# CESNET/UltraGrid

Hardware: AMD Instinct MI355X
Metric: Mpixels/s encode (UYVY->DXT5-YCoCg, 4K) (higher is better)
Workload: dtype f32

## Files before the change

### include/ug_mi355x.h

```cpp
#ifndef UG_MI355X_H
#define UG_MI355X_H

#include <stddef.h>
#include <stdint.h>

#ifdef __cplusplus
extern "C" {
#endif

#define UG_HIP_ABI_VERSION 5

#define UG_HIP_SUCCESS      0
#define UG_HIP_EINVAL     (-1)
#define UG_HIP_EUNSUPP    (-2)
#define UG_HIP_ERUNTIME   (-3)

typedef void *ug_hip_stream_t;

typedef enum {
        UG_PF_NONE = 0,
        UG_PF_RGBA = 1,
        UG_PF_UYVY = 2,
        UG_PF_YUYV = 3,
        UG_PF_RGB  = 4,
// ... 61 lines not shown
                                   float *ms_per_launch);

#define UG_DXT_TIES_EVEN    0
#define UG_DXT_TIES_AWAY    1
#define UG_DXT_TIES_DEFAULT UG_DXT_TIES_EVEN

int ug_hip_dxt_encode(ug_pixfmt_t in, ug_dxt_t out, const void *src_dev, void *dst_dev,
                      int width, int height, int src_pitch, ug_hip_stream_t stream);
int ug_hip_dxt_encode_batch(ug_pixfmt_t in, ug_dxt_t out, const void *src_dev, void *dst_dev,
                            int width, int height, int src_pitch, int frames,
                            size_t src_frame_stride, size_t dst_frame_stride,
                            ug_hip_stream_t stream);
int ug_hip_dxt_encode_batch_ex(ug_pixfmt_t in, ug_dxt_t out, const void *src_dev, void *dst_dev,
                               int width, int height, int src_pitch, int frames,
                               size_t src_frame_stride, size_t dst_frame_stride, int ties,
                               ug_hip_stream_t stream);
size_t ug_hip_dxt_size(ug_dxt_t out, int width, int height);

int ug_hip_rgb_to_dxt1(const void *src, void *out, int size_x, int size_y, ug_hip_stream_t stream);
int ug_hip_yuv_to_dxt1(const void *src, void *out, int size_x, int size_y, ug_hip_stream_t stream);
int ug_hip_rgb_to_dxt6(const void *src, void *out, int size_x, int size_y, ug_hip_stream_t stream);
int ug_hip_yuv_to_dxt6(const void *src, void *out, int size_x, int size_y, ug_hip_stream_t stream);
int ug_hip_yuv422_to_yuv444(const void *src, void *out, int pix_count, ug_hip_stream_t stream);

int ug_hip_dxt_decode(ug_dxt_t in, ug_pixfmt_t out, const void *src_dev, void *dst_dev, int width, int height,
                      int dst_pitch, int rshift, int gshift, int bshift, ug_hip_stream_t stream);
int ug_hip_dxt_decode_ex(ug_dxt_t in, ug_pixfmt_t out, const void *src_dev, void *dst_dev, int width, int height,
                         int dst_pitch, int rshift, int gshift, int bshift, int ties, ug_hip_stream_t stream);
int ug_hip_selftest_dxt_decode(unsigned *mismatches, ug_hip_stream_t stream);
int ug_hip_dxt_decode_debug(int mode, unsigned *flagged_blocks_dev);
int ug_hip_selftest_dxt_encode(unsigned *mismatches, ug_hip_stream_t stream);
int ug_hip_dxt_encode_stats(unsigned long long full_form_waves[2], int reset);
int ug_hip_dxt_encode_stats_ex(unsigned long long *counts, int n, int reset);
typedef struct ug_hip_ldgm ug_hip_ldgm;
int ug_hip_ldgm_stats(const ug_hip_ldgm *s, int *launches, int *copies, int *levels);

int  ug_hip_ldgm_create(int device, int k, int m, const int *pcm, int w_f, ug_hip_ldgm **out);
void ug_hip_ldgm_destroy(ug_hip_ldgm *s);
int  ug_hip_ldgm_encode(ug_hip_ldgm *s, void *buf_dev, int ps, ug_hip_stream_t stream);
int  ug_hip_ldgm_decode(ug_hip_ldgm *s, void *buf_dev, int ps, const uint8_t *received, uint8_t *recovered, int *all_data_known,
                        ug_hip_stream_t stream);
int  ug_hip_ldgm_encode_host(ug_hip_ldgm *s, void *buf_host, int ps, ug_hip_stream_t stream);
int  ug_hip_ldgm_decode_host(ug_hip_ldgm *s, void *buf_host, int ps, const uint8_t *received, uint8_t *recovered, int *all_data_known,
                             ug_hip_stream_t stream);

int ug_hip_pixfmt_supported(ug_pixfmt_t in, ug_pixfmt_t out);
int ug_hip_pixfmt_best(ug_pixfmt_t in, const ug_pixfmt_t *candidates, ug_pixfmt_t *out);
int ug_hip_pixfmt_convert(ug_pixfmt_t in, ug_pixfmt_t out, const void *src_dev, void *dst_dev,
                          int width, int height, int src_pitch, int dst_pitch,
                          int rshift, int gshift, int bshift, ug_hip_stream_t stream);
int ug_hip_pixfmt_convert_batch(ug_pixfmt_t in, ug_pixfmt_t out, const void *src_dev, void *dst_dev, int width, int height,
                                int src_pitch, int dst_pitch, int rshift, int gshift, int bshift, int frames,
                                size_t src_frame_stride, size_t dst_frame_stride, ug_hip_stream_t stream);
int ug_hip_pixfmt_line_func(const char *func, const void *src_dev, void *dst_dev, int width, int height, int src_pitch, int dst_pitch, int dst_len,
                            int rshift, int gshift, int bshift, ug_hip_stream_t stream);
int ug_hip_linesize(ug_pixfmt_t fmt, int width);
int ug_hip_deinterlace_blend(void *frame_dev, size_t linesize, int lines, ug_hip_stream_t stream);
int ug_hip_deinterlace_blend_batch(void *frame_dev, size_t linesize, int lines, int frames, size_t frame_stride, ug_hip_stream_t stream);

struct ug_scale_desc {
        const void *src;
        void       *dst;
        ug_pixfmt_t format;
        int         interlaced_merged;
        int         src_width, src_height, dst_width, dst_height;
        size_t      src_pitch, dst_pitch;
// ... 162 lines not shown
```

### ultragrid_amd/csrc/dxt_encode.hip

```cpp
#include "ug_common.h"

#ifndef UG_DXT_TBUF
#define UG_DXT_TBUF 1
#endif

namespace {

constexpr float kInv255  = 0.00392156862745f;
constexpr float kOffset  = (float) (128.0 / 255.0);
constexpr float kInsetC  = (float) ((8.0 / 255.0) / 16.0);
constexpr float kInsetY  = (float) ((16.0 / 255.0) / 32.0);

__device__ __forceinline__ float clamp01(float v) { return fminf(1.0f, fmaxf(0.0f, v)); }

template <bool AWAY>
__device__ __forceinline__ uint32_t round_u32(float x)
{
        if (!AWAY) {
                return (uint32_t) rintf(x);
        }
        const uint32_t r = (uint32_t) (x + 0.5f);
        return x < 0.5f ? 0u : r;
}

constexpr uint32_t kDiv14Exact = 0x0d800000u;
__device__ __forceinline__ float div14(float x)
{
        constexpr float rc = 1.0f / 14.0f;
        const float q = x * rc;
        const float r = __builtin_fmaf(-q, 14.0f, x);
        return __builtin_fmaf(r, rc, q);
}

// ... 45 lines not shown
        x = (x | (x << 1)) & 0x55555555u;
        return x;
}

#ifndef UG_DXT_NO_FAST_INDEX
#define UG_DXT_FAST_INDEX 1
#else
#define UG_DXT_FAST_INDEX 0
#endif
#ifndef UG_DXT1_FAST_GROUP
#define UG_DXT1_FAST_GROUP 2
#endif
#ifndef UG_DXT5_FAST_GROUP
#define UG_DXT5_FAST_GROUP 4
#endif
#ifndef UG_DXT5_ALPHA_GROUP
#define UG_DXT5_ALPHA_GROUP 8
#endif
#ifndef UG_DXT_PAIR_ZONE
#define UG_DXT_PAIR_ZONE 1
#endif
#ifndef UG_DXT_BITS_INDEX
#define UG_DXT_BITS_INDEX 1
#endif
#ifndef UG_DXT_PAIR_COV
#define UG_DXT_PAIR_COV 1
#endif
#ifndef UG_DXT_POW2_FOLD
#define UG_DXT_POW2_FOLD 1
#endif
#ifndef UG_DXT_PAIR_LINEAR
#define UG_DXT_PAIR_LINEAR 1
#endif
[[maybe_unused]] constexpr float kIndexBias = 8388608.0f;
[[maybe_unused]] constexpr uint32_t kIndexBits = 0x4b000000u;
constexpr uint32_t index_bias_sum(int fields, int shift)
{
        uint32_t s = 0;
        for (int n = 0; n < fields && n * shift < 32; n++) s += kIndexBits << (n * shift);
        return s;
}
__device__ unsigned long long g_full_form_waves[2];
__device__ __forceinline__ void count_full_form(int which)
{
        if ((int) threadIdx.x == __builtin_amdgcn_readfirstlane((int) threadIdx.x)) {
                atomicAdd(&g_full_form_waves[which], 1ull);
        }
}
__device__ unsigned long long g_exact_cov_waves;
__device__ __forceinline__ void count_exact_cov()
{
        if ((int) threadIdx.x == __builtin_amdgcn_readfirstlane((int) threadIdx.x)) {
                atomicAdd(&g_exact_cov_waves, 1ull);
        }
}
constexpr int kPairSlots = 256, kPairSlotStride = 16;
__device__ unsigned long long g_exact_pair_waves[kPairSlots * kPairSlotStride];
__device__ __forceinline__ void count_exact_pair()
{
        if ((int) threadIdx.x == __builtin_amdgcn_readfirstlane((int) threadIdx.x)) {
                const uint32_t slot = ((blockIdx.x + 17u * blockIdx.y + 101u * blockIdx.z) * 4u + threadIdx.y) & (kPairSlots - 1);
                atomicAdd(&g_exact_pair_waves[slot * kPairSlotStride], 1ull);
        }
}
struct IndexTables {
        float *alpha;
        float4 *colour;
};

struct Px16 {
        float a[16], b[16], c[16];
};

__device__ __forceinline__ void yuv_pair_to_rgb(float y0, float y1, float u, float v, Px16 &p, int i)
{
        const float U = u - 0.5f, V = v - 0.5f;
        const float rv = 1.7926f * V, gu = 0.2132f * U, gv = 0.5328f * V, bu = 2.1124f * U;
        const float Y0 = 1.1643f * (y0 - 0.0625f), Y1 = 1.1643f * (y1 - 0.0625f);
        p.a[i] = Y0 + rv;
        p.b[i] = (Y0 - gu) - gv;
        p.c[i] = Y0 + bu;
        p.a[i + 1] = Y1 + rv;
        p.b[i + 1] = (Y1 - gu) - gv;
        p.c[i + 1] = Y1 + bu;
}

__device__ __forceinline__ float byte_f(uint32_t w, int k) { return (float) ((w >> (8 * k)) & 0xffu) * kInv255; }

__device__ __forceinline__ void row_rgb(const uint32_t *w, Px16 &p, int i)
{
        p.a[i + 0] = byte_f(w[0], 0); p.b[i + 0] = byte_f(w[0], 1); p.c[i + 0] = byte_f(w[0], 2);
        p.a[i + 1] = byte_f(w[0], 3); p.b[i + 1] = byte_f(w[1], 0); p.c[i + 1] = byte_f(w[1], 1);
        p.a[i + 2] = byte_f(w[1], 2); p.b[i + 2] = byte_f(w[1], 3); p.c[i + 2] = byte_f(w[2], 0);
        p.a[i + 3] = byte_f(w[2], 1); p.b[i + 3] = byte_f(w[2], 2); p.c[i + 3] = byte_f(w[2], 3);
}

template <int IN>
// ... 293 lines not shown
        }
        __device__ __forceinline__ float samp(int r, int s) const
        {
                return (float) ((w[r][s / 3] >> (10 * (s % 3) + 2)) & 0xffu) * kInv255;
        }
        __device__ __forceinline__ void block(int k, Px16 &p) const
        {
#pragma unroll
                for (int r = 0; r < 4; r++) {
#pragma unroll
                        for (int pr = 0; pr < 2; pr++) {
                                const int s = 8 * k + 4 * pr;
                                yuv_pair_to_rgb(samp(r, s + 1), samp(r, s + 3), samp(r, s), samp(r, s + 2), p, 4 * r + 2 * pr);
                        }
                }
        }
        __device__ __forceinline__ void block_edge(int k, Px16 &p, bool half) const
        {
#pragma unroll
                for (int r = 0; r < 4; r++) {
                        const int s = 8 * k;
                        const float u0 = samp(r, s), y00 = samp(r, s + 1), v0 = samp(r, s + 2), y01 = samp(r, s + 3);
                        yuv_pair_to_rgb(y00, y01, u0, v0, p, 4 * r);
                        const float u1 = half ? u0 : samp(r, s + 4), y10 = half ? y01 : samp(r, s + 5), v1 = half ? v0 : samp(r, s + 6), y11 = half ? y01 : samp(r, s + 7);
                        yuv_pair_to_rgb(y10, y11, u1, v1, p, 4 * r + 2);
                }
        }
};

template <bool AWAY, bool PAIRS>
__device__ __forceinline__ uint4 encode_dxt5ycocg(Px16 &p, const IndexTables &tab)
{
        constexpr bool kFold = UG_DXT_POW2_FOLD;
#pragma unroll
        for (int i = 0; i < 16; i++) {
                const float r = p.a[i], g = p.b[i], b = p.c[i];
                const float t = __builtin_fmaf(g, 2.0f, r);
                p.a[i] = kFold ? t + b : (t + b) * 0.25f;
                p.b[i] = __builtin_fmaf(r - b, 0.5f, kOffset);
                p.c[i] = __builtin_fmaf(__builtin_fmaf(g, 2.0f, -r) - b, 0.25f, kOffset);
        }
        float *Y = p.a, *Co = p.b, *Cg = p.c;

        float mnY = Y[0], mxY = Y[0], mnCo = Co[0], mxCo = Co[0], mnCg = Cg[0], mxCg = Cg[0];
#pragma unroll
        for (int i = 1; i < 16; i++) {
                mnY = fminf(mnY, Y[i]);    mxY = fmaxf(mxY, Y[i]);
                mnCo = fminf(mnCo, Co[i]); mxCo = fmaxf(mxCo, Co[i]);
                mnCg = fminf(mnCg, Cg[i]); mxCg = fmaxf(mxCg, Cg[i]);
        }

        if constexpr (!(PAIRS && UG_DXT_PAIR_COV)) {
                const float midx = (mxCo + mnCo) * 0.5f, midy = (mxCg + mnCg) * 0.5f;
                float cov = 0.0f;
#pragma unroll
                for (int i = 0; i < 16; i++) {
                        const float tx = Co[i] - midx, ty = Cg[i] - midy;
                        cov = cov + tx * ty;
                }
                if (cov < 0.0f) {
                        const float t = mxCg; mxCg = mnCg; mnCg = t;
                }
        } else {
                const float midx = (mxCo + mnCo) * 0.5f, midy = (mxCg + mnCg) * 0.5f;
                const float hx = mxCo - mnCo, hy = mxCg - mnCg;
                float rough = 0.0f;
#pragma unroll
                for (int i = 0; i < 16; i += 2) {
                        rough = __builtin_fmaf(Co[i] - midx, Cg[i] - midy, rough);
                }
                const lanemask_t certain = LANEMASK(fabsf(rough) > 0.5e-5f * __builtin_fmaf(hx, hy, hx + hy)) | LANEMASK(hx * hy == 0.0f);
                bool swap;
                if (__builtin_expect(certain == LANEMASK(true), 1)) {
                        swap = rough < 0.0f;
                } else {
                        float mx = midx, my = midy;
                        asm volatile("; exact covariance" : "+v"(mx), "+v"(my) :: "memory");
                        count_exact_cov();
                        float cov = 0.0f;
#pragma unroll
                        for (int i = 0; i < 16; i++) {
                                const float tx = Co[i] - mx, ty = Cg[i] - my;
                                cov = cov + tx * ty;
                        }
                        swap = cov < 0.0f;
                }
                if (swap) {
                        const float t = mxCg; mxCg = mnCg; mnCg = t;
                }
        }

        uint32_t scale = 1;
        float fs = 1.0f, rfs = 1.0f;
        {
                const float m0 = fmaxf(fabsf(mnCo - kOffset), fabsf(mnCg - kOffset));
                const float m1 = fmaxf(fabsf(mxCo - kOffset), fabsf(mxCg - kOffset));
                const float m = fmaxf(m0, m1);
                if (m < (float) (64.0 / 255.0)) { scale = 2; fs = 2.0f; rfs = 0.5f; }
                if (m < (float) (32.0 / 255.0)) { scale = 4; fs = 4.0f; rfs = 0.25f; }
        }

        uint32_t w_end;
        float cmx[2], cmn[2];
        {
                const float q[2] = { 31.0f, 63.0f };
                const float mx_in[2] = { mxCo, mxCg }, mn_in[2] = { mnCo, mnCg };
                uint32_t imax[2], imin[2];
#pragma unroll
                for (int k = 0; k < 2; k++) {
                        float a = kFold ? __builtin_fmaf(mx_in[k] - kOffset, fs, kOffset) : (mx_in[k] - kOffset) * fs + kOffset;
                        float b = kFold ? __builtin_fmaf(mn_in[k] - kOffset, fs, kOffset) : (mn_in[k] - kOffset) * fs + kOffset;
                        const float inset = kFold ? __builtin_fmaf(a - b, 0.0625f, -kInsetC) : (a - b) * 0.0625f - kInsetC;
                        b = clamp01(b + inset);
                        a = clamp01(a - inset);
                        imax[k] = round_u32<AWAY>(a * q[k]);
                        imin[k] = round_u32<AWAY>(b * q[k]);
                }
                w_end = ((imax[0] << 11) | (imax[1] << 5) | (scale - 1)) |
                        (((imin[0] << 11) | (imin[1] << 5) | (scale - 1)) << 16);
                imax[0] = (imax[0] << 3) | (imax[0] >> 2);
                imax[1] = (imax[1] << 2) | (imax[1] >> 4);
                imin[0] = (imin[0] << 3) | (imin[0] >> 2);
                imin[1] = (imin[1] << 2) | (imin[1] >> 4);
                const float inv255 = (float) (1.0 / 255.0);
#pragma unroll
                for (int k = 0; k < 2; k++) {
                        cmx[k] = kFold ? __builtin_fmaf((float) imax[k] * inv255 - kOffset, rfs, kOffset) : ((float) imax[k] * inv255 - kOffset) * rfs + kOffset;
                        cmn[k] = kFold ? __builtin_fmaf((float) imin[k] * inv255 - kOffset, rfs, kOffset) : ((float) imin[k] * inv255 - kOffset) * rfs + kOffset;
                }
        }

        if constexpr (kFold) {
                const float inset = __builtin_fmaf(mxY - mnY, 0.0078125f, -kInsetY);
                mnY = clamp01(__builtin_fmaf(mnY, 0.25f, inset));
                mxY = clamp01(__builtin_fmaf(mxY, 0.25f, -inset));
        } else {
                const float inset = (mxY - mnY) * 0.03125f - kInsetY;
                mnY = clamp01(mnY + inset);
                mxY = clamp01(mxY - inset);
        }
        uint32_t w0 = (round_u32<AWAY>(mnY * 255.0f) << 8) | round_u32<AWAY>(mxY * 255.0f);
        uint32_t w1 = 0;
        {
                const float inv7 = (float) (1.0 / 7.0);
                const float range = mxY - mnY;
#ifdef UG_DXT_IEEE_DIV14
                const float mid = range / 14.0f;
#else
                float mid = div14(range);
                if (__builtin_expect(__any((__float_as_uint(range) - 1u) < (kDiv14Exact - 1u)), 0)) {
                        mid = range / 14.0f;
                }
#endif
                float ab[8];
                if constexpr (kFold) {
                        ab[1] = __builtin_fmaf(mid, 4.0f, mnY * 4.0f);
#pragma unroll
                        for (int k = 2; k <= 7; k++) {
                                const float cx_ = (float) (4 * (8 - k)), cn_ = (float) (4 * (k - 1));
                                const float sum = k <= 3 || k == 5 ? __builtin_fmaf(mnY, cn_, cx_ * mxY) : __builtin_fmaf(mxY, cx_, cn_ * mnY);
                                ab[k] = __builtin_fmaf(mid, 4.0f, sum * inv7);
// ... 89 lines not shown
                                for (int k = 1; k <= 7; k++) {
                                        c += (a <= ab[k]) ? 1u : 0u;
                                }
                                uint32_t &acc = i >= 10 ? hi : lo;
                                acc = (acc << 3) | c;
                        }
                }
                auto map_fields = [](uint32_t w) {
                        const uint32_t M = 0x09249249u;
                        const uint32_t c0 = w & M, c1 = (w >> 1) & M, c2 = (w >> 2) & M;
                        const uint32_t t = c1 & c0;
                        const uint32_t i0 = ((c0 ^ M) & (c1 | c2)) | (t & c2);
                        const uint32_t i1 = c1 ^ c0, i2 = c2 ^ t;
                        return i0 | (i1 << 1) | (i2 << 2);
                };
                lo = map_fields(lo);
                hi = map_fields(hi);
                w0 |= lo << 16;
                w1 = (lo >> 16) | (hi << 14);
        }
        uint32_t w_cidx = 0;
        {
                const float q1 = (float) (1.0 / 3.0), q2 = (float) (2.0 / 3.0);
                const float w1 = 1.0f - q1, w2 = 1.0f - q2;
                float cx[4], cy[4];
                cx[0] = cmx[0]; cy[0] = cmx[1];
                cx[1] = cmn[0]; cy[1] = cmn[1];
                cx[2] = lerp_w(cx[0], cx[1], w1, q1); cy[2] = lerp_w(cy[0], cy[1], w1, q1);
                cx[3] = lerp_w(cx[0], cx[1], w2, q2); cy[3] = lerp_w(cy[0], cy[1], w2, q2);
#if UG_DXT_FAST_INDEX
                const float vx = cx[1] - cx[0], vy = cy[1] - cy[0];
                const float vv = vx * vx + vy * vy;
                const float e0 = fmaxf(fmaxf(mxCo, cx[0]), cx[1]) - fminf(fminf(mnCo, cx[0]), cx[1]);
                const float e1 = fmaxf(fmaxf(fmaxf(mxCg, mnCg), cy[0]), cy[1]) - fminf(fminf(fminf(mxCg, mnCg), cy[0]), cy[1]);
                const float dmax = e0 * e0 + e1 * e1;
                const bool flat = (mnCo == mxCo) & (mnCg == mxCg);
                if (__builtin_expect(__all(((vv >= 1e-5f) & (vv * 256.0f > dmax)) | flat), 1)) {
                        float4 *const tc = tab.colour;
                        constexpr bool kLinear = PAIRS && UG_DXT_PAIR_ZONE && UG_DXT_PAIR_LINEAR;
                        auto write_rows = [&](float ax, float ay, float bx, float by, float cx2, float cy2, float cx3, float cy3) {
                                tc[0 * 64] = make_float4(ax, ay, cx2, cy2);
                                tc[1 * 64] = make_float4(cx2, cy2, cx3, cy3);
                                tc[2 * 64] = make_float4(bx, by, cx3, cy3);
                        };
                        if constexpr (kLinear) {
                                auto linear_row = [&](int a, int b) {
                                        const float mx = cx[a] - cx[b], my = cy[a] - cy[b], sx = cx[a] + cx[b], sy = cy[a] + cy[b];
                                        return make_float4(mx, my, 0.5f * __builtin_fmaf(mx, sx, my * sy), 0.0f);
                                };
                                tc[0 * 64] = linear_row(0, 2);
                                tc[1 * 64] = linear_row(2, 3);
                                tc[2 * 64] = linear_row(1, 3);
                        } else {
                                write_rows(cx[0], cy[0], cx[1], cy[1], cx[2], cy[2], cx[3], cy[3]);
                        }
#if UG_DXT_BITS_INDEX
                        const float inv = 1.5f * __builtin_amdgcn_rcpf(vv);
                        const float ka = vx * inv, kb = vy * inv;
                        const float kc = kFold ? __builtin_fmaf(-cx[0], ka, __builtin_fmaf(-cy[0], kb, -0.25f)) : -(cx[0] * ka + cy[0] * kb) - 0.25f;
#else
                        const float inv = __builtin_amdgcn_rcpf(vv);
                        const float ka = vx * inv, kb = vy * inv;
                        const float kc = -(cx[0] * ka + cy[0] * kb);
#endif
                        uint32_t zones = 0, open = 0;
                        constexpr int kC = UG_DXT5_FAST_GROUP, kGroups = 16 / kC;
                        constexpr int kP = PAIRS && UG_DXT_PAIR_ZONE ? 2 : 1;
// ... 37 lines not shown
                                        } else {
                                                const float ax = Co[i] - q.x, ay = Cg[i] - q.y, bx = Co[i] - q.z, by = Cg[i] - q.w;
                                                const float da = ax * ax + ay * ay, db = bx * bx + by * by;
                                                if (j % kP == 0) {
                                                        zones = (zones << (2 * kP)) + kk[slot][j / kP];
                                                }
                                                open = shift_in(open, LANEMASK(da > db));
                                        }
                                }
                                if constexpr (kLinear) {
                                        static_assert(kC / kP == 2, "two pairs per group");
                                        least = fminf(fminf(least, mag[0]), mag[1]);
                                }
                                __builtin_amdgcn_sched_barrier(0);
                        }
#if UG_DXT_BITS_INDEX
                        zones -= index_bias_sum(16 / kP, 2 * kP);
#endif
                        if (kP == 2) {
                                zones |= zones << 2;
                        }
                        uint32_t c;
                        if constexpr (kLinear) {
                                const float eps = __builtin_fmaf(dmax, 4.76837158203125e-07f, 1e-6f * __builtin_amdgcn_sqrtf(vv));
                                const lanemask_t certain = LANEMASK(least > eps) | LANEMASK(flat);
                                if (__builtin_expect(certain == LANEMASK(true), 1)) {
                                        c = (open | (open << 12)) & 0x000f000fu;
                                        c = (c | (c << 6)) & 0x03030303u;
                                        c = (c | (c << 3)) & 0x11111111u;
                                        c |= c << 2;
                                } else {
                                        asm volatile("; per-pixel distances" ::: "memory");
                                        count_exact_pair();
                                        write_rows(cx[0], cy[0], cx[1], cy[1], cx[2], cy[2], cx[3], cy[3]);
                                        open = 0;
#pragma unroll
                                        for (int i = 15; i >= 0; i--) {
                                                const float4 q = *(const float4 *) ((const char *) tc + (((zones >> (2 * i)) & 3u) << 10));
                                                const float ax = Co[i] - q.x, ay = Cg[i] - q.y, bx = Co[i] - q.z, by = Cg[i] - q.w;
                                                const float da = ax * ax + ay * ay, db = bx * bx + by * by;
                                                open = shift_in(open, LANEMASK(da > db));
                                        }
                                        c = spread16(open);
                                }
                        } else {
                                c = spread16(open);
                        }
                        const uint32_t k0 = zones & 0x55555555u, k1 = (zones >> 1) & 0x55555555u;
                        w_cidx = ((k0 & c) | k1) | ((k0 | c) << 1);
                        if (__any(flat)) {
                                asm volatile("; flat blocks" ::: "memory");
                                float4 p02, p13;
                                if constexpr (kLinear) {
                                        p02 = make_float4(cx[0], cy[0], cx[2], cy[2]); p13 = make_float4(cx[1], cy[1], cx[3], cy[3]);
                                } else {
                                        p02 = tc[0 * 64]; p13 = tc[2 * 64];
                                }
                                const float px[4] = { p02.x, p13.x, p02.z, p13.z }, py[4] = { p02.y, p13.y, p02.w, p13.w };
                                float d[4];
#pragma unroll
                                for (int k = 0; k < 4; k++) {
                                        const float tx = Co[0] - px[k], ty = Cg[0] - py[k];
                                        d[k] = tx * tx + ty * ty;
                                }
                                w_cidx = flat ? palette_index(d[0], d[1], d[2], d[3]) * 0x55555555u : w_cidx;
                        }
                } else
#endif
                {
                asm volatile("; colour index full form" ::: "memory");
#if UG_DXT_FAST_INDEX
                count_full_form(0);
#endif
                f32x2 cx2[4], cy2[4];
#pragma unroll
                for (int k = 0; k < 4; k++) {
                        cx2[k] = (f32x2) { cx[k], cx[k] };
                        cy2[k] = (f32x2) { cy[k], cy[k] };
                }
#pragma unroll
                for (int i = 14; i >= 0; i -= 2) {
                        const f32x2 co = { Co[i], Co[i + 1] }, cg = { Cg[i], Cg[i + 1] };
                        f32x2 d[4];
#pragma unroll
                        for (int k = 0; k < 4; k++) {
                                const f32x2 tx = co - cx2[k], ty = cg - cy2[k];
                                d[k] = tx * tx + ty * ty;
                        }
#pragma unroll
                        for (int h = 1; h >= 0; h--) {
                                const float d0 = d[0][h], d1 = d[1][h], d2 = d[2][h], d3 = d[3][h];
                                const lanemask_t b0 = LANEMASK(d0 > d3), b1 = LANEMASK(d1 > d2), b2 = LANEMASK(d0 > d2),
                                                 b3 = LANEMASK(d1 > d3), b4 = LANEMASK(d2 > d3);
                                w_cidx = shift_in(w_cidx, (b1 & b2) | (b0 & b3));
                                w_cidx = shift_in(w_cidx, b0 & b4);
                        }
                }
                }
        }

        return make_uint4(w0, w1, w_end, w_cidx);
}

template <bool AWAY>
__device__ __forceinline__ uint2 encode_dxt1(const Px16 &p, const IndexTables &tab)
{
// ... 451 lines not shown
                           int src_pitch, int frames, size_t sfs, size_t dfs, int iters, ug_hip_stream_t stream,
                           float *ms_per_launch)
{
        if (!ms_per_launch || iters <= 0) return UG_HIP_EINVAL;
        hipStream_t st = (hipStream_t) stream;
        int rc = ug_hip_dxt_encode_batch(in, out, src, dst, width, height, src_pitch, frames, sfs, dfs, stream);
        if (rc != UG_HIP_SUCCESS) return rc;
        hipEvent_t e0, e1;
        UG_HIP_TRY(hipEventCreate(&e0));
        UG_HIP_TRY(hipEventCreate(&e1));
        {
                (void) hipEventRecord(e0, st);
                for (int i = 0; i < iters && rc == UG_HIP_SUCCESS; i++) {
                        rc = ug_hip_dxt_encode_batch(in, out, src, dst, width, height, src_pitch, frames, sfs, dfs, stream);
                }
                (void) hipEventRecord(e1, st);
                hipError_t e = hipEventSynchronize(e1);
                if (e != hipSuccess) {
                        ug::set_last_error(e, "hipEventSynchronize");
                        rc = UG_HIP_ERUNTIME;
                } else {
                        float ms = 0;
                        (void) hipEventElapsedTime(&ms, e0, e1);
                        *ms_per_launch = ms / iters;
                }
        }
        (void) hipEventDestroy(e0);
        (void) hipEventDestroy(e1);
        return rc;
}

}

extern "C" int ug_hip_dxt_encode_stats(unsigned long long full_form_waves[2], int reset)
{
        UG_HIP_TRY(hipDeviceSynchronize());
        if (full_form_waves) {
                UG_HIP_TRY(hipMemcpyFromSymbol(full_form_waves, HIP_SYMBOL(g_full_form_waves), 2 * sizeof(unsigned long long)));
        }
        if (reset) {
                const unsigned long long zero[2] = { 0, 0 };
                UG_HIP_TRY(hipMemcpyToSymbol(HIP_SYMBOL(g_full_form_waves), zero, sizeof zero));
                UG_HIP_TRY(hipMemcpyToSymbol(HIP_SYMBOL(g_exact_cov_waves), zero, sizeof zero[0]));
                static const unsigned long long no_pairs[kPairSlots * kPairSlotStride] = {};
                UG_HIP_TRY(hipMemcpyToSymbol(HIP_SYMBOL(g_exact_pair_waves), no_pairs, sizeof no_pairs));
        }
        return UG_HIP_SUCCESS;
}

extern "C" int ug_hip_dxt_encode_stats_ex(unsigned long long *counts, int n, int reset)
{
        if (n < 0 || n > 4 || (n > 0 && !counts)) return UG_HIP_EINVAL;
        unsigned long long all[4] = { 0, 0, 0, 0 };
        UG_HIP_TRY(hipDeviceSynchronize());
        if (n > 0) {
                UG_HIP_TRY(hipMemcpyFromSymbol(all, HIP_SYMBOL(g_full_form_waves), 2 * sizeof all[0]));
                UG_HIP_TRY(hipMemcpyFromSymbol(all + 2, HIP_SYMBOL(g_exact_cov_waves), sizeof all[0]));
                static unsigned long long pairs[kPairSlots * kPairSlotStride];
                UG_HIP_TRY(hipMemcpyFromSymbol(pairs, HIP_SYMBOL(g_exact_pair_waves), sizeof pairs));
                for (int i = 0; i < kPairSlots; i++) all[3] += pairs[i * kPairSlotStride];
                for (int i = 0; i < n; i++) counts[i] = all[i];
        }
        return reset ? ug_hip_dxt_encode_stats(nullptr, 1) : UG_HIP_SUCCESS;
}

extern "C" int ug_hip_selftest_dxt_encode(unsigned *mismatches, ug_hip_stream_t stream)
{
        if (!mismatches) return UG_HIP_EINVAL;
        unsigned *dev = nullptr;
        UG_HIP_TRY(hipMalloc((void **) &dev, sizeof *dev));
        hipStream_t st = (hipStream_t) stream;
        hipError_t err = hipMemsetAsync(dev, 0, sizeof *dev, st);
        if (err == hipSuccess) {
                hipLaunchKernelGGL(selftest_div14_kernel, dim3((0x3f800000u >> 8) + 1), dim3(256), 0, st, dev);
                err = hipGetLastError();
        }
        if (err == hipSuccess) err = hipMemcpyAsync(mismatches, dev, sizeof *dev, hipMemcpyDeviceToHost, st);
        if (err == hipSuccess) err = hipStreamSynchronize(st);
        (void) hipFree(dev);
        if (err != hipSuccess) {
                ug::set_last_error(err, "ug_hip_selftest_dxt_encode");
                return UG_HIP_ERUNTIME;
        }
        return UG_HIP_SUCCESS;
}
```

### ultragrid_amd/lib.py

```python
from __future__ import annotations

import ctypes as C
import os

_HERE = os.path.dirname(os.path.abspath(__file__))
LIB_PATH = os.environ.get("UG_MI355X_LIB") or os.path.join(_HERE, "libug_mi355x.so")

PF_NONE, PF_RGBA, PF_UYVY, PF_YUYV, PF_RGB, PF_BGR, PF_V210, PF_RG48, PF_YUV444, PF_UYVY_RAW, PF_I420 = range(11)
PF_R10K, PF_R12L, PF_Y216, PF_Y416, PF_VUYA, PF_DVS10 = range(11, 17)
PF_UYVY_GL = 17
PF_NAMES = {"RGBA": PF_RGBA, "UYVY": PF_UYVY, "YUYV": PF_YUYV, "RGB": PF_RGB, "BGR": PF_BGR, "v210": PF_V210,
            "RG48": PF_RG48, "YUV444": PF_YUV444, "UYVY_RAW": PF_UYVY_RAW, "R10k": PF_R10K, "R12L": PF_R12L, "Y216": PF_Y216,
            "Y416": PF_Y416, "VUYA": PF_VUYA, "DVS10": PF_DVS10}
DXT1, DXT1_YUV, DXT5_YCOCG = 1, 2, 6
TIES_EVEN, TIES_AWAY = 0, 1
JPEG_CS_ASIS, JPEG_CS_RGB, JPEG_CS_YCBCR_BT601, JPEG_CS_YCBCR_BT601_256LVLS, JPEG_CS_YCBCR_BT709 = 0, 1, 2, 3, 4
JPEG_NONINTERLEAVED = 1
JPEG_INPUT_UYVY = 2
JPEG_INPUT_RGB = 4
COPY_NO_WAIT, COPY_NO_JOIN = 1, 2
ABI_VERSION = 5

SUCCESS, EINVAL, EUNSUPP, ERUNTIME = 0, -1, -2, -3

# ... 29 lines not shown
    "ug_hip_device_numa_node": (_i, [_i, C.POINTER(_i)]),
    "ug_hip_bind_thread_to_device": (_i, [_i, C.POINTER(_i)]),
    "ug_hip_numa_node_of_pci": (_i, [C.c_char_p, C.c_char_p, C.POINTER(_i)]),
    "ug_hip_bind_thread_to_numa_node": (_i, [_i, C.c_char_p, C.POINTER(_i)]),
    "ug_hip_time_dxt_encode": (_i, [_i, _i, _vp, _vp, _i, _i, _i, _i, _sz, _sz, _i, _vp, C.POINTER(C.c_float)]),
    "ug_hip_dxt_encode": (_i, [_i, _i, _vp, _vp, _i, _i, _i, _vp]),
    "ug_hip_dxt_encode_batch": (_i, [_i, _i, _vp, _vp, _i, _i, _i, _i, _sz, _sz, _vp]),
    "ug_hip_dxt_encode_batch_ex": (_i, [_i, _i, _vp, _vp, _i, _i, _i, _i, _sz, _sz, _i, _vp]),
    "ug_hip_dxt_size": (_sz, [_i, _i, _i]),
    "ug_hip_rgb_to_dxt1": (_i, [_vp, _vp, _i, _i, _vp]),
    "ug_hip_yuv_to_dxt1": (_i, [_vp, _vp, _i, _i, _vp]),
    "ug_hip_rgb_to_dxt6": (_i, [_vp, _vp, _i, _i, _vp]),
    "ug_hip_yuv_to_dxt6": (_i, [_vp, _vp, _i, _i, _vp]),
    "ug_hip_yuv422_to_yuv444": (_i, [_vp, _vp, _i, _vp]),
    "ug_hip_dxt_decode": (_i, [_i, _i, _vp, _vp, _i, _i, _i, _i, _i, _i, _vp]),
    "ug_hip_dxt_decode_ex": (_i, [_i, _i, _vp, _vp, _i, _i, _i, _i, _i, _i, _i, _vp]),
    "ug_hip_pixfmt_supported": (_i, [_i, _i]),
    "ug_hip_pixfmt_convert": (_i, [_i, _i, _vp, _vp, _i, _i, _i, _i, _i, _i, _i, _vp]),
    "ug_hip_pixfmt_convert_batch": (_i, [_i, _i, _vp, _vp, _i, _i, _i, _i, _i, _i, _i, _i, _sz, _sz, _vp]),
    "ug_hip_linesize": (_i, [_i, _i]),
    "ug_hip_deinterlace_blend": (_i, [_vp, _sz, _i, _vp]),
    "ug_hip_deinterlace_blend_batch": (_i, [_vp, _sz, _i, _i, _sz, _vp]),
    "ug_hip_uyvy_to_i420": (_i, [_vp, _i, _vp, _i, _vp, _i, _vp, _i, _i, _i, _vp]),
    "ug_hip_v210_to_p010le": (_i, [_vp, _i, _vp, _i, _vp, _i, _i, _i, _vp]),
    "ug_hip_yuv420p_to_uyvy": (_i, [_vp, _i, _vp, _i, _vp, _i, _vp, _i, _i, _i, _vp]),
    "ug_hip_yuv422p_to_uyvy": (_i, [_vp, _i, _vp, _i, _vp, _i, _vp, _i, _i, _i, _vp]),
    "ug_hip_yuv422p10le_to_v210": (_i, [_vp, _i, _vp, _i, _vp, _i, _vp, _i, _i, _i, _vp]),
    "ug_hip_uyvy_to_i422": (_i, [_vp, _i, _vp, _i, _vp, _i, _vp, _i, _i, _i, _vp]),
    "ug_hip_selftest_dxt_decode": (_i, [C.POINTER(C.c_uint), _vp]),
    "ug_hip_dxt_decode_debug": (_i, [_i, _vp]),
    "ug_hip_selftest_dxt_encode": (_i, [C.POINTER(C.c_uint), _vp]),
    "ug_hip_dxt_encode_stats": (_i, [C.POINTER(C.c_ulonglong), _i]),
    "ug_hip_dxt_encode_stats_ex": (_i, [C.POINTER(C.c_ulonglong), _i, _i]),
    "ug_hip_ldgm_stats": (_i, [_vp, C.POINTER(_i), C.POINTER(_i), C.POINTER(_i)]),
    "ug_hip_ldgm_create": (_i, [_i, _i, _i, _vp, _i, C.POINTER(_vp)]),
    "ug_hip_ldgm_destroy": (None, [_vp]),
    "ug_hip_ldgm_encode": (_i, [_vp, _vp, _i, _vp]),
    "ug_hip_ldgm_decode": (_i, [_vp, _vp, _i, _vp, _vp, C.POINTER(_i), _vp]),
    "ug_hip_ldgm_encode_host": (_i, [_vp, _vp, _i, _vp]),
    "ug_hip_ldgm_decode_host": (_i, [_vp, _vp, _i, _vp, _vp, C.POINTER(_i), _vp]),
    "ug_hip_uyvy_to_nv12": (_i, [_vp, _i, _vp, _i, _vp, _i, _i, _i, _vp]),
    "ug_hip_pixfmt_best": (_i, [_i, C.POINTER(_i), C.POINTER(_i)]),
    "ug_hip_pixfmt_line_func": (_i, [C.c_char_p, _vp, _vp, _i, _i, _i, _i, _i, _i, _i, _i, _vp]),
    "ug_hip_from_planar": (_i, [C.c_char_p, _vp, _vp]),
    "ug_hip_to_planar": (_i, [C.c_char_p, _vp, _vp]),
    "ug_hip_from_planar_supported": (_i, [C.c_char_p]),
    "ug_hip_to_planar_supported": (_i, [C.c_char_p]),
    "ug_hip_uv_to_av": (_i, [C.c_char_p, C.c_char_p, _vp, _vp, _vp]),
    "ug_hip_av_to_uv": (_i, [C.c_char_p, C.c_char_p, _vp, _i, _vp, C.POINTER(_i), _vp]),
    "ug_hip_uv_to_av_supported": (_i, [C.c_char_p, C.c_char_p]),
    "ug_hip_av_to_uv_supported": (_i, [C.c_char_p, C.c_char_p]),
    "ug_hip_color_coeffs": (_i, [_i, _i, C.POINTER(_i)]),
    "ug_hip_compute_color_coeffs": (_i, [C.c_double, C.c_double, _i, C.POINTER(_i)]),
    "ug_hip_jpeg_qtable": (None, [_i, _i, _vp]),
    "ug_hip_jpeg_divisors": (None, [_vp, _vp]),
    "ug_hip_jpeg_fdct_quant_plane": (_i, [_vp, _i, _i, _i, _i, _i, _vp, _vp, _vp, _vp]),
    "ug_hip_uyvy_to_jpeg420_coeffs": (_i, [_vp, _i, _i, _i, _vp, _vp, _vp, _vp, _vp]),
    "ug_hip_uyvy_to_jpeg422_coeffs": (_i, [_vp, _i, _i, _i, _vp, _vp, _vp, _vp, _vp]),
    "ug_hip_uyvy_to_jpeg42x_coeffs_batch": (_i, [_i, _vp, _i, _i, _i, _vp, _vp, _vp, _vp, _i, _sz, _sz, _sz, _vp]),
    "ug_hip_jpeg_encoder_create": (_i, [_i, _i, _i, _i, C.POINTER(_vp)]),
    "ug_hip_jpeg_encoder_create_sub": (_i, [_i, _i, _i, _i, _i, C.POINTER(_vp)]),
    "ug_hip_jpeg_encoder_create_ex": (_i, [_i, _i, _i, _i, _i, _i, _i, C.POINTER(_vp)]),
    "ug_hip_jpeg_colour_matrix": (_i, [_i, _i, C.POINTER(C.c_float)]),
    "ug_hip_jpeg_colour_convert": (_i, [_i, _i, _i, _vp, _i, _vp, _i, _i, _i, _vp]),
    "ug_hip_jpeg_encoder_destroy": (None, [_vp]),
    "ug_hip_jpeg_encoder_max_size": (_sz, [_vp]),
# ... 75 lines not shown
```

Before: 960,600.

## Derive DXT5-YCoCg chroma box from even pixels with certified fallback to full box

For the paired DXT5-YCoCg path, the colour conversion defers the Co/Cg offset and scale on odd pixels, and the chroma bounding box, diagonal and scale are computed from the eight even pixels only. A certification mask checks margins on the covariance sign, the scale thresholds and endpoint rounding ties. Any wave with an uncertain lane finishes the odd pixels and recomputes the full sixteen-pixel box, diagonal and endpoints, and the later exact paths also finalise the odd pixels on demand. The wave counters are also sharded into strided slots to reduce atomic contention. This cuts min/max and FMA work in the common case, at the cost of extra branches, register pressure and a correctness dependence on the tolerance constants.

```diff
diff --git a/include/ug_mi355x.h b/include/ug_mi355x.h
--- a/include/ug_mi355x.h
+++ b/include/ug_mi355x.h
@@ -117,6 +117,7 @@
 int ug_hip_selftest_dxt_encode(unsigned *mismatches, ug_hip_stream_t stream);
 int ug_hip_dxt_encode_stats(unsigned long long full_form_waves[2], int reset);
 int ug_hip_dxt_encode_stats_ex(unsigned long long *counts, int n, int reset);
+int ug_hip_dxt_encode_stats_box(unsigned long long *waves, int reset);
 typedef struct ug_hip_ldgm ug_hip_ldgm;
 int ug_hip_ldgm_stats(const ug_hip_ldgm *s, int *launches, int *copies, int *levels);
 
diff --git a/ultragrid_amd/csrc/dxt_encode.hip b/ultragrid_amd/csrc/dxt_encode.hip
--- a/ultragrid_amd/csrc/dxt_encode.hip
+++ b/ultragrid_amd/csrc/dxt_encode.hip
@@ -1,4 +1,5 @@
 #include "ug_common.h"
+#include <type_traits>
 
 #ifndef UG_DXT_TBUF
 #define UG_DXT_TBUF 1
@@ -110,6 +111,10 @@
 #ifndef UG_DXT_PAIR_LINEAR
 #define UG_DXT_PAIR_LINEAR 1
 #endif
+#ifndef UG_DXT_PAIR_BOX
+#define UG_DXT_PAIR_BOX 1
+#endif
+[[maybe_unused]] constexpr float kBoxTie = 1.2e-6f, kBoxScale = 2e-6f, kBoxSpread = 4e-6f;
 [[maybe_unused]] constexpr float kIndexBias = 8388608.0f;
 [[maybe_unused]] constexpr uint32_t kIndexBits = 0x4b000000u;
 constexpr uint32_t index_bias_sum(int fields, int shift)
@@ -118,6 +123,23 @@
         for (int n = 0; n < fields && n * shift < 32; n++) s += kIndexBits << (n * shift);
         return s;
 }
+constexpr int kPairSlots = 256, kPairSlotStride = 16;
+constexpr int kWaveCounter = kPairSlots * kPairSlotStride;
+__device__ __forceinline__ void count_wave(unsigned long long *counter)
+{
+        if ((int) threadIdx.x == __builtin_amdgcn_readfirstlane((int) threadIdx.x)) {
+                const uint32_t slot = ((blockIdx.x + 17u * blockIdx.y + 101u * blockIdx.z) * 4u + (uint32_t) __builtin_amdgcn_readfirstlane((int) threadIdx.y)) & (kPairSlots - 1);
+                atomicAdd(&counter[slot * kPairSlotStride], 1ull);
+        }
+}
+#if UG_DXT_PAIR_BOX
+__device__ unsigned long long g_full_form_waves[2][kWaveCounter];
+__device__ __forceinline__ void count_full_form(int which) { count_wave(g_full_form_waves[which]); }
+__device__ unsigned long long g_exact_cov_waves[kWaveCounter];
+__device__ __forceinline__ void count_exact_cov() { count_wave(g_exact_cov_waves); }
+__device__ unsigned long long g_exact_pair_waves[kWaveCounter];
+__device__ __forceinline__ void count_exact_pair() { count_wave(g_exact_pair_waves); }
+#else
 __device__ unsigned long long g_full_form_waves[2];
 __device__ __forceinline__ void count_full_form(int which)
 {
@@ -132,7 +154,6 @@
                 atomicAdd(&g_exact_cov_waves, 1ull);
         }
 }
-constexpr int kPairSlots = 256, kPairSlotStride = 16;
 __device__ unsigned long long g_exact_pair_waves[kPairSlots * kPairSlotStride];
 __device__ __forceinline__ void count_exact_pair()
 {
@@ -141,6 +162,9 @@
                 atomicAdd(&g_exact_pair_waves[slot * kPairSlotStride], 1ull);
         }
 }
+#endif
+__device__ unsigned long long g_box_waves[kWaveCounter];
+[[maybe_unused]] __device__ __forceinline__ void count_box() { count_wave(g_box_waves); }
 struct IndexTables {
         float *alpha;
         float4 *colour;
@@ -500,24 +524,90 @@
 __device__ __forceinline__ uint4 encode_dxt5ycocg(Px16 &p, const IndexTables &tab)
 {
         constexpr bool kFold = UG_DXT_POW2_FOLD;
+        constexpr bool kBox = PAIRS && UG_DXT_PAIR_BOX && UG_DXT_PAIR_COV && UG_DXT_PAIR_ZONE && UG_DXT_PAIR_LINEAR && UG_DXT_FAST_INDEX;
 #pragma unroll
         for (int i = 0; i < 16; i++) {
                 const float r = p.a[i], g = p.b[i], b = p.c[i];
                 const float t = __builtin_fmaf(g, 2.0f, r);
                 p.a[i] = kFold ? t + b : (t + b) * 0.25f;
-                p.b[i] = __builtin_fmaf(r - b, 0.5f, kOffset);
-                p.c[i] = __builtin_fmaf(__builtin_fmaf(g, 2.0f, -r) - b, 0.25f, kOffset);
+                if (!kBox || i % 2 == 0) {
+                        p.b[i] = __builtin_fmaf(r - b, 0.5f, kOffset);
+                        p.c[i] = __builtin_fmaf(__builtin_fmaf(g, 2.0f, -r) - b, 0.25f, kOffset);
+                } else {
+                        p.b[i] = r - b;
+                        p.c[i] = __builtin_fmaf(g, 2.0f, -r) - b;
+                }
         }
         float *Y = p.a, *Co = p.b, *Cg = p.c;
+        [[maybe_unused]] bool have_odd = !kBox;
+        [[maybe_unused]] auto need_odd = [&]() {
+                if constexpr (kBox) {
+                        if (!have_odd) {
+#pragma unroll
+                                for (int i = 1; i < 16; i += 2) {
+                                        Co[i] = __builtin_fmaf(Co[i], 0.5f, kOffset);
+                                        Cg[i] = __builtin_fmaf(Cg[i], 0.25f, kOffset);
+                                }
+                                have_odd = true;
+                        }
+                }
+        };
 
         float mnY = Y[0], mxY = Y[0], mnCo = Co[0], mxCo = Co[0], mnCg = Cg[0], mxCg = Cg[0];
 #pragma unroll
         for (int i = 1; i < 16; i++) {
                 mnY = fminf(mnY, Y[i]);    mxY = fmaxf(mxY, Y[i]);
-                mnCo = fminf(mnCo, Co[i]); mxCo = fmaxf(mxCo, Co[i]);
-                mnCg = fminf(mnCg, Cg[i]); mxCg = fmaxf(mxCg, Cg[i]);
-        }
-
+                if (!kBox || i % 2 == 0) {
+                        mnCo = fminf(mnCo, Co[i]); mxCo = fmaxf(mxCo, Co[i]);
+                        mnCg = fminf(mnCg, Cg[i]); mxCg = fmaxf(mxCg, Cg[i]);
+                }
+        }
+
+        if constexpr (kBox) {
+                asm volatile("" : "+v"(mnY), "+v"(mxY));
+        }
+
+        [[maybe_unused]] lanemask_t box_certain = LANEMASK(true);
+        [[maybe_unused]] lanemask_t luma_flat_certain = 0;
+        [[maybe_unused]] float loCg = mnCg, hiCg = mxCg;
+        [[maybe_unused]] auto pair_diagonal = [&](auto on_even_box) {
+                if constexpr (kBox) {
+                        constexpr bool kEvenBox = decltype(on_even_box)::value;
+                        const float midx = (mxCo + mnCo) * 0.5f, midy = (mxCg + mnCg) * 0.5f;
+                        const float hx = mxCo - mnCo, hy = mxCg - mnCg;
+                        float rough = 0.0f;
+#pragma unroll
+                        for (int i = 0; i < 16; i += 2) {
+                                rough = __builtin_fmaf(Co[i] - midx, Cg[i] - midy, rough);
+                        }
+                        bool swap;
+                        if constexpr (kEvenBox) {
+                                const lanemask_t decided = LANEMASK(fabsf(rough) > 0.5e-5f * __builtin_fmaf(hx, hy, hx + hy));
+                                box_certain = decided & LANEMASK(fminf(hx, hy) > kBoxSpread);
+                                luma_flat_certain = LANEMASK(mnY == mxY) & (decided | LANEMASK(hx * hy == 0.0f));
+                                swap = rough < 0.0f;
+                        } else {
+                                const lanemask_t certain = LANEMASK(fabsf(rough) > 0.5e-5f * __builtin_fmaf(hx, hy, hx + hy)) | LANEMASK(hx * hy == 0.0f);
+                                if (__builtin_expect(certain == LANEMASK(true), 1)) {
+                                        swap = rough < 0.0f;
+                                } else {
+                                        float mx = midx, my = midy;
+                                        asm volatile("; exact covariance" : "+v"(mx), "+v"(my) :: "memory");
+                                        count_exact_cov();
+                                        float cov = 0.0f;
+#pragma unroll
+                                        for (int i = 0; i < 16; i++) {
+                                                const float tx = Co[i] - mx, ty = Cg[i] - my;
+                                                cov = cov + tx * ty;
+                                        }
+                                        swap = cov < 0.0f;
+                                }
+                        }
+                        if (swap) {
+                                const float t = mxCg; mxCg = mnCg; mnCg = t;
+                        }
+                }
+        };
         if constexpr (!(PAIRS && UG_DXT_PAIR_COV)) {
                 const float midx = (mxCo + mnCo) * 0.5f, midy = (mxCg + mnCg) * 0.5f;
                 float cov = 0.0f;
@@ -530,71 +620,136 @@
                         const float t = mxCg; mxCg = mnCg; mnCg = t;
                 }
         } else {
-                const float midx = (mxCo + mnCo) * 0.5f, midy = (mxCg + mnCg) * 0.5f;
-                const float hx = mxCo - mnCo, hy = mxCg - mnCg;
-                float rough = 0.0f;
-#pragma unroll
-                for (int i = 0; i < 16; i += 2) {
-                        rough = __builtin_fmaf(Co[i] - midx, Cg[i] - midy, rough);
-                }
-                const lanemask_t certain = LANEMASK(fabsf(rough) > 0.5e-5f * __builtin_fmaf(hx, hy, hx + hy)) | LANEMASK(hx * hy == 0.0f);
-                bool swap;
-                if (__builtin_expect(certain == LANEMASK(true), 1)) {
-                        swap = rough < 0.0f;
+                if constexpr (kBox) {
+                        pair_diagonal(std::true_type());
                 } else {
-                        float mx = midx, my = midy;
-                        asm volatile("; exact covariance" : "+v"(mx), "+v"(my) :: "memory");
-                        count_exact_cov();
-                        float cov = 0.0f;
-#pragma unroll
-                        for (int i = 0; i < 16; i++) {
-                                const float tx = Co[i] - mx, ty = Cg[i] - my;
-                                cov = cov + tx * ty;
-                        }
-                        swap = cov < 0.0f;
-                }
-                if (swap) {
-                        const float t = mxCg; mxCg = mnCg; mnCg = t;
+                        const float midx = (mxCo + mnCo) * 0.5f, midy = (mxCg + mnCg) * 0.5f;
+                        const float hx = mxCo - mnCo, hy = mxCg - mnCg;
+                        float rough = 0.0f;
+#pragma unroll
+                        for (int i = 0; i < 16; i += 2) {
+                                rough = __builtin_fmaf(Co[i] - midx, Cg[i] - midy, rough);
+                        }
+                        const lanemask_t certain = LANEMASK(fabsf(rough) > 0.5e-5f * __builtin_fmaf(hx, hy, hx + hy)) | LANEMASK(hx * hy == 0.0f);
+                        bool swap;
+                        if (__builtin_expect(certain == LANEMASK(true), 1)) {
+                                swap = rough < 0.0f;
+                        } else {
+                                float mx = midx, my = midy;
+                                asm volatile("; exact covariance" : "+v"(mx), "+v"(my) :: "memory");
+                                count_exact_cov();
+                                float cov = 0.0f;
+#pragma unroll
+                                for (int i = 0; i < 16; i++) {
+                                        const float tx = Co[i] - mx, ty = Cg[i] - my;
+                                        cov = cov + tx * ty;
+                                }
+                                swap = cov < 0.0f;
+                        }
+                        if (swap) {
+                                const float t = mxCg; mxCg = mnCg; mnCg = t;
+                        }
                 }
         }
 
         uint32_t scale = 1;
         float fs = 1.0f, rfs = 1.0f;
-        {
-                const float m0 = fmaxf(fabsf(mnCo - kOffset), fabsf(mnCg - kOffset));
-                const float m1 = fmaxf(fabsf(mxCo - kOffset), fabsf(mxCg - kOffset));
-                const float m = fmaxf(m0, m1);
-                if (m < (float) (64.0 / 255.0)) { scale = 2; fs = 2.0f; rfs = 0.5f; }
-                if (m < (float) (32.0 / 255.0)) { scale = 4; fs = 4.0f; rfs = 0.25f; }
-        }
-
         uint32_t w_end;
         float cmx[2], cmn[2];
-        {
-                const float q[2] = { 31.0f, 63.0f };
-                const float mx_in[2] = { mxCo, mxCg }, mn_in[2] = { mnCo, mnCg };
-                uint32_t imax[2], imin[2];
-#pragma unroll
-                for (int k = 0; k < 2; k++) {
-                        float a = kFold ? __builtin_fmaf(mx_in[k] - kOffset, fs, kOffset) : (mx_in[k] - kOffset) * fs + kOffset;
-                        float b = kFold ? __builtin_fmaf(mn_in[k] - kOffset, fs, kOffset) : (mn_in[k] - kOffset) * fs + kOffset;
-                        const float inset = kFold ? __builtin_fmaf(a - b, 0.0625f, -kInsetC) : (a - b) * 0.0625f - kInsetC;
-                        b = clamp01(b + inset);
-                        a = clamp01(a - inset);
-                        imax[k] = round_u32<AWAY>(a * q[k]);
-                        imin[k] = round_u32<AWAY>(b * q[k]);
-                }
-                w_end = ((imax[0] << 11) | (imax[1] << 5) | (scale - 1)) |
-                        (((imin[0] << 11) | (imin[1] << 5) | (scale - 1)) << 16);
-                imax[0] = (imax[0] << 3) | (imax[0] >> 2);
-                imax[1] = (imax[1] << 2) | (imax[1] >> 4);
-                imin[0] = (imin[0] << 3) | (imin[0] >> 2);
-                imin[1] = (imin[1] << 2) | (imin[1] >> 4);
-                const float inv255 = (float) (1.0 / 255.0);
-#pragma unroll
-                for (int k = 0; k < 2; k++) {
-                        cmx[k] = kFold ? __builtin_fmaf((float) imax[k] * inv255 - kOffset, rfs, kOffset) : ((float) imax[k] * inv255 - kOffset) * rfs + kOffset;
-                        cmn[k] = kFold ? __builtin_fmaf((float) imin[k] * inv255 - kOffset, rfs, kOffset) : ((float) imin[k] * inv255 - kOffset) * rfs + kOffset;
+        if constexpr (!kBox) {
+                {
+                        const float m0 = fmaxf(fabsf(mnCo - kOffset), fabsf(mnCg - kOffset));
+                        const float m1 = fmaxf(fabsf(mxCo - kOffset), fabsf(mxCg - kOffset));
+                        const float m = fmaxf(m0, m1);
+                        if (m < (float) (64.0 / 255.0)) { scale = 2; fs = 2.0f; rfs = 0.5f; }
+                        if (m < (float) (32.0 / 255.0)) { scale = 4; fs = 4.0f; rfs = 0.25f; }
+                }
+                {
+                        const float q[2] = { 31.0f, 63.0f };
+                        const float mx_in[2] = { mxCo, mxCg }, mn_in[2] = { mnCo, mnCg };
+                        uint32_t imax[2], imin[2];
+#pragma unroll
+                        for (int k = 0; k < 2; k++) {
+                                float a = kFold ? __builtin_fmaf(mx_in[k] - kOffset, fs, kOffset) : (mx_in[k] - kOffset) * fs + kOffset;
+                                float b = kFold ? __builtin_fmaf(mn_in[k] - kOffset, fs, kOffset) : (mn_in[k] - kOffset) * fs + kOffset;
+                                const float inset = kFold ? __builtin_fmaf(a - b, 0.0625f, -kInsetC) : (a - b) * 0.0625f - kInsetC;
+                                b = clamp01(b + inset);
+                                a = clamp01(a - inset);
+                                imax[k] = round_u32<AWAY>(a * q[k]);
+                                imin[k] = round_u32<AWAY>(b * q[k]);
+                        }
+                        w_end = ((imax[0] << 11) | (imax[1] << 5) | (scale - 1)) |
+                                (((imin[0] << 11) | (imin[1] << 5) | (scale - 1)) << 16);
+                        imax[0] = (imax[0] << 3) | (imax[0] >> 2);
+                        imax[1] = (imax[1] << 2) | (imax[1] >> 4);
+                        imin[0] = (imin[0] << 3) | (imin[0] >> 2);
+                        imin[1] = (imin[1] << 2) | (imin[1] >> 4);
+                        const float inv255 = (float) (1.0 / 255.0);
+#pragma unroll
+                        for (int k = 0; k < 2; k++) {
+                                cmx[k] = kFold ? __builtin_fmaf((float) imax[k] * inv255 - kOffset, rfs, kOffset) : ((float) imax[k] * inv255 - kOffset) * rfs + kOffset;
+                                cmn[k] = kFold ? __builtin_fmaf((float) imin[k] * inv255 - kOffset, rfs, kOffset) : ((float) imin[k] * inv255 - kOffset) * rfs + kOffset;
+                        }
+                }
+        } else {
+                auto scale_and_end_points = [&](auto certify) -> lanemask_t {
+                        constexpr bool kCertify = decltype(certify)::value;
+                        [[maybe_unused]] lanemask_t covered = 0;
+                        scale = 1; fs = 1.0f; rfs = 1.0f;
+                        const float m0 = fmaxf(fabsf(mnCo - kOffset), fabsf(mnCg - kOffset));
+                        const float m1 = fmaxf(fabsf(mxCo - kOffset), fabsf(mxCg - kOffset));
+                        const float m = fmaxf(m0, m1);
+                        if (m < (float) (64.0 / 255.0)) { scale = 2; fs = 2.0f; rfs = 0.5f; }
+                        if (m < (float) (32.0 / 255.0)) { scale = 4; fs = 4.0f; rfs = 0.25f; }
+                        if constexpr (kCertify) {
+                                covered = LANEMASK(fabsf(m - (float) (64.0 / 255.0)) > kBoxScale) & LANEMASK(fabsf(m - (float) (32.0 / 255.0)) > kBoxScale);
+                        }
+                        const float q[2] = { 31.0f, 63.0f };
+                        const float mx_in[2] = { mxCo, mxCg }, mn_in[2] = { mnCo, mnCg };
+                        uint32_t imax[2], imin[2];
+#pragma unroll
+                        for (int k = 0; k < 2; k++) {
+                                float a = kFold ? __builtin_fmaf(mx_in[k] - kOffset, fs, kOffset) : (mx_in[k] - kOffset) * fs + kOffset;
+                                float b = kFold ? __builtin_fmaf(mn_in[k] - kOffset, fs, kOffset) : (mn_in[k] - kOffset) * fs + kOffset;
+                                const float inset = kFold ? __builtin_fmaf(a - b, 0.0625f, -kInsetC) : (a - b) * 0.0625f - kInsetC;
+                                b = clamp01(b + inset);
+                                a = clamp01(a - inset);
+                                imax[k] = round_u32<AWAY>(a * q[k]);
+                                imin[k] = round_u32<AWAY>(b * q[k]);
+                                if constexpr (kCertify) {
+                                        const float xa = a * q[k], xb = b * q[k];
+                                        covered &= LANEMASK(fmaxf(fabsf(xa - rintf(xa)), fabsf(xb - rintf(xb))) < __builtin_fmaf(fs, -q[k] * kBoxTie, 0.5f));
+                                }
+                        }
+                        w_end = ((imax[0] << 11) | (imax[1] << 5) | (scale - 1)) |
+                                (((imin[0] << 11) | (imin[1] << 5) | (scale - 1)) << 16);
+                        imax[0] = (imax[0] << 3) | (imax[0] >> 2);
+                        imax[1] = (imax[1] << 2) | (imax[1] >> 4);
+                        imin[0] = (imin[0] << 3) | (imin[0] >> 2);
+                        imin[1] = (imin[1] << 2) | (imin[1] >> 4);
+                        const float inv255 = (float) (1.0 / 255.0);
+#pragma unroll
+                        for (int k = 0; k < 2; k++) {
+                                cmx[k] = kFold ? __builtin_fmaf((float) imax[k] * inv255 - kOffset, rfs, kOffset) : ((float) imax[k] * inv255 - kOffset) * rfs + kOffset;
+                                cmn[k] = kFold ? __builtin_fmaf((float) imin[k] * inv255 - kOffset, rfs, kOffset) : ((float) imin[k] * inv255 - kOffset) * rfs + kOffset;
+                        }
+                        return covered;
+                };
+                box_certain = (box_certain & scale_and_end_points(std::true_type())) | luma_flat_certain;
+                if (__builtin_expect(box_certain != LANEMASK(true), 0)) {
+                        asm volatile("; sixteen-pixel box" ::: "memory");
+                        count_box();
+                        need_odd();
+                        mnCo = fminf(mnCo, Co[1]); mxCo = fmaxf(mxCo, Co[1]);
+                        mnCg = fminf(loCg, Cg[1]); mxCg = fmaxf(hiCg, Cg[1]);
+#pragma unroll
+                        for (int i = 3; i < 16; i += 2) {
+                                mnCo = fminf(mnCo, Co[i]); mxCo = fmaxf(mxCo, Co[i]);
+                                mnCg = fminf(mnCg, Cg[i]); mxCg = fmaxf(mxCg, Cg[i]);
+                        }
+                        loCg = mnCg; hiCg = mxCg;
+                        pair_diagonal(std::false_type());
+                        scale_and_end_points(std::false_type());
                 }
         }
 
@@ -750,7 +905,8 @@
                 const float vx = cx[1] - cx[0], vy = cy[1] - cy[0];
                 const float vv = vx * vx + vy * vy;
                 const float e0 = fmaxf(fmaxf(mxCo, cx[0]), cx[1]) - fminf(fminf(mnCo, cx[0]), cx[1]);
-                const float e1 = fmaxf(fmaxf(fmaxf(mxCg, mnCg), cy[0]), cy[1]) - fminf(fminf(fminf(mxCg, mnCg), cy[0]), cy[1]);
+                const float e1 = kBox ? fmaxf(fmaxf(hiCg, cy[0]), cy[1]) - fminf(fminf(loCg, cy[0]), cy[1])
+                                      : fmaxf(fmaxf(fmaxf(mxCg, mnCg), cy[0]), cy[1]) - fminf(fminf(fminf(mxCg, mnCg), cy[0]), cy[1]);
                 const float dmax = e0 * e0 + e1 * e1;
                 const bool flat = (mnCo == mxCo) & (mnCg == mxCg);
                 if (__builtin_expect(__all(((vv >= 1e-5f) & (vv * 256.0f > dmax)) | flat), 1)) {
@@ -854,6 +1010,7 @@
                                 } else {
                                         asm volatile("; per-pixel distances" ::: "memory");
                                         count_exact_pair();
+                                        need_odd();
                                         write_rows(cx[0], cy[0], cx[1], cy[1], cx[2], cy[2], cx[3], cy[3]);
                                         open = 0;
 #pragma unroll
@@ -894,6 +1051,7 @@
 #if UG_DXT_FAST_INDEX
                 count_full_form(0);
 #endif
+                need_odd();
                 f32x2 cx2[4], cy2[4];
 #pragma unroll
                 for (int k = 0; k < 4; k++) {
@@ -1411,18 +1569,44 @@
 
 }
 
+static int dxt_encode_counters(unsigned long long all[5])
+{
+        static unsigned long long slots[kWaveCounter];
+        auto sum = [&](const void *symbol, size_t offset, unsigned long long &out) -> hipError_t {
+                const hipError_t e = hipMemcpyFromSymbol(slots, symbol, sizeof slots, offset);
+                out = 0;
+                for (int i = 0; i < kPairSlots; i++) out += slots[i * kPairSlotStride];
+                return e;
+        };
+#if UG_DXT_PAIR_BOX
+        UG_HIP_TRY(sum(HIP_SYMBOL(g_full_form_waves), 0, all[0]));
+        UG_HIP_TRY(sum(HIP_SYMBOL(g_full_form_waves), sizeof slots, all[1]));
+        UG_HIP_TRY(sum(HIP_SYMBOL(g_exact_cov_waves), 0, all[2]));
+#else
+        UG_HIP_TRY(hipMemcpyFromSymbol(all, HIP_SYMBOL(g_full_form_waves), 2 * sizeof all[0]));
+        UG_HIP_TRY(hipMemcpyFromSymbol(all + 2, HIP_SYMBOL(g_exact_cov_waves), sizeof all[0]));
+#endif
+        UG_HIP_TRY(sum(HIP_SYMBOL(g_exact_pair_waves), 0, all[3]));
+        UG_HIP_TRY(sum(HIP_SYMBOL(g_box_waves), 0, all[4]));
+        return UG_HIP_SUCCESS;
+}
+
 extern "C" int ug_hip_dxt_encode_stats(unsigned long long full_form_waves[2], int reset)
 {
         UG_HIP_TRY(hipDeviceSynchronize());
         if (full_form_waves) {
-                UG_HIP_TRY(hipMemcpyFromSymbol(full_form_waves, HIP_SYMBOL(g_full_form_waves), 2 * sizeof(unsigned long long)));
+                unsigned long long all[5];
+                const int rc = dxt_encode_counters(all);
+                if (rc != UG_HIP_SUCCESS) return rc;
+                full_form_waves[0] = all[0];
+                full_form_waves[1] = all[1];
         }
         if (reset) {
-                const unsigned long long zero[2] = { 0, 0 };
-                UG_HIP_TRY(hipMemcpyToSymbol(HIP_SYMBOL(g_full_form_waves), zero, sizeof zero));
-                UG_HIP_TRY(hipMemcpyToSymbol(HIP_SYMBOL(g_exact_cov_waves), zero, sizeof zero[0]));
-                static const unsigned long long no_pairs[kPairSlots * kPairSlotStride] = {};
-                UG_HIP_TRY(hipMemcpyToSymbol(HIP_SYMBOL(g_exact_pair_waves), no_pairs, sizeof no_pairs));
+                static const unsigned long long zero[2 * kWaveCounter] = {};
+                UG_HIP_TRY(hipMemcpyToSymbol(HIP_SYMBOL(g_full_form_waves), zero, sizeof g_full_form_waves));
+                UG_HIP_TRY(hipMemcpyToSymbol(HIP_SYMBOL(g_exact_cov_waves), zero, sizeof g_exact_cov_waves));
+                UG_HIP_TRY(hipMemcpyToSymbol(HIP_SYMBOL(g_exact_pair_waves), zero, sizeof g_exact_pair_waves));
+                UG_HIP_TRY(hipMemcpyToSymbol(HIP_SYMBOL(g_box_waves), zero, sizeof g_box_waves));
         }
         return UG_HIP_SUCCESS;
 }
@@ -1430,15 +1614,24 @@
 extern "C" int ug_hip_dxt_encode_stats_ex(unsigned long long *counts, int n, int reset)
 {
         if (n < 0 || n > 4 || (n > 0 && !counts)) return UG_HIP_EINVAL;
-        unsigned long long all[4] = { 0, 0, 0, 0 };
         UG_HIP_TRY(hipDeviceSynchronize());
         if (n > 0) {
-                UG_HIP_TRY(hipMemcpyFromSymbol(all, HIP_SYMBOL(g_full_form_waves), 2 * sizeof all[0]));
-                UG_HIP_TRY(hipMemcpyFromSymbol(all + 2, HIP_SYMBOL(g_exact_cov_waves), sizeof all[0]));
-                static unsigned long long pairs[kPairSlots * kPairSlotStride];
-                UG_HIP_TRY(hipMemcpyFromSymbol(pairs, HIP_SYMBOL(g_exact_pair_waves), sizeof pairs));
-                for (int i = 0; i < kPairSlots; i++) all[3] += pairs[i * kPairSlotStride];
+                unsigned long long all[5];
+                const int rc = dxt_encode_counters(all);
+                if (rc != UG_HIP_SUCCESS) return rc;
                 for (int i = 0; i < n; i++) counts[i] = all[i];
+        }
+        return reset ? ug_hip_dxt_encode_stats(nullptr, 1) : UG_HIP_SUCCESS;
+}
+
+extern "C" int ug_hip_dxt_encode_stats_box(unsigned long long *waves, int reset)
+{
+        UG_HIP_TRY(hipDeviceSynchronize());
+        if (waves) {
+                unsigned long long all[5];
+                const int rc = dxt_encode_counters(all);
+                if (rc != UG_HIP_SUCCESS) return rc;
+                *waves = all[4];
         }
         return reset ? ug_hip_dxt_encode_stats(nullptr, 1) : UG_HIP_SUCCESS;
 }
diff --git a/ultragrid_amd/lib.py b/ultragrid_amd/lib.py
--- a/ultragrid_amd/lib.py
+++ b/ultragrid_amd/lib.py
@@ -85,6 +85,7 @@
     "ug_hip_selftest_dxt_encode": (_i, [C.POINTER(C.c_uint), _vp]),
     "ug_hip_dxt_encode_stats": (_i, [C.POINTER(C.c_ulonglong), _i]),
     "ug_hip_dxt_encode_stats_ex": (_i, [C.POINTER(C.c_ulonglong), _i, _i]),
+    "ug_hip_dxt_encode_stats_box": (_i, [C.POINTER(C.c_ulonglong), _i]),
     "ug_hip_ldgm_stats": (_i, [_vp, C.POINTER(_i), C.POINTER(_i), C.POINTER(_i)]),
     "ug_hip_ldgm_create": (_i, [_i, _i, _i, _vp, _i, C.POINTER(_vp)]),
     "ug_hip_ldgm_destroy": (None, [_vp]),
```

Result: faster. 970,900 (median of 6 runs) (+1.1%).
